# facebookresearch/actionmesh

Hardware: NVIDIA H100
Metric: denoiser_steps_per_sec (higher is better)
Workload: dtype bf16

## Files before the change

actionmesh_b200/csrc/attention.cu:

```cuda
#include "common.cuh"
#include "ptx.cuh"
#include "attention.cuh"

namespace amb {

constexpr int ATT_BQ = 128;
constexpr int ATT_BK = 128;
constexpr int ATT_THREADS = 384;
constexpr int ATT_STAGES = 2;

template <int D>
struct AttnSmem {
  static constexpr int BOX_BYTES = 128 * 128;
  static constexpr int Q_BYTES = (D / 64) * BOX_BYTES;
  static constexpr int KV_BYTES = (D / 64) * BOX_BYTES;
  static constexpr int Q_OFF = 0;
  static constexpr int K_OFF = Q_BYTES;
  static constexpr int V_OFF = K_OFF + ATT_STAGES * KV_BYTES;
  static constexpr int BAR_OFF = V_OFF + ATT_STAGES * KV_BYTES;
  static constexpr int NUM_BARS = 1 + 4 * ATT_STAGES;
  static constexpr int TOTAL = BAR_OFF + NUM_BARS * 8 + 1024;
};

template <int D>
__device__ __forceinline__ void qk_issue(float* sc, uint32_t sq_addr, uint32_t sk_addr) {
#pragma unroll
  for (int k = 0; k < D / 16; ++k) {
    const uint32_t off = (k >> 2) * AttnSmem<D>::BOX_BYTES + (k & 3) * 32;
    wgmma_ss_n128(sc, make_desc_kmajor_sw128(sq_addr + off), make_desc_kmajor_sw128(sk_addr + off), k > 0 ? 1u : 0u);
  }
  wgmma_commit();
}

template <int D>
__device__ __forceinline__ void pv_issue(float* o, const uint32_t* pk, uint32_t sv_addr) {
#pragma unroll
  for (int kk = 0; kk < ATT_BK / 16; ++kk) {
    const uint64_t vdesc = make_desc_mnmajor_sw128(sv_addr + kk * 2048, AttnSmem<D>::BOX_BYTES);
    if constexpr (D == 128) wgmma_rs_n128_tb(o, pk + 4 * kk, vdesc, 1u);
    else wgmma_rs_n64_tb(o, pk + 4 * kk, vdesc, 1u);
  }
  wgmma_commit();
}

__device__ __forceinline__ void softmax_tile(float* sc, int valid, int q, float c, float& m_a, float& m_b, float& l_a,
                                             float& l_b, float& al_a, float& al_b) {
  if (valid < ATT_BK) {
#pragma unroll
    for (int i = 0; i < 16; ++i) {
      const int key = 8 * i + 2 * q;
      if (key >= valid) sc[4 * i] = sc[4 * i + 2] = -INFINITY;
      if (key + 1 >= valid) sc[4 * i + 1] = sc[4 * i + 3] = -INFINITY;
    }
  }
  float mx_a = m_a, mx_b = m_b;
#pragma unroll
  for (int i = 0; i < 16; ++i) {
    mx_a = fmaxf(mx_a, fmaxf(sc[4 * i], sc[4 * i + 1]));
    mx_b = fmaxf(mx_b, fmaxf(sc[4 * i + 2], sc[4 * i + 3]));
  }
  mx_a = fmaxf(mx_a, __shfl_xor_sync(0xffffffffu, mx_a, 1));
  mx_b = fmaxf(mx_b, __shfl_xor_sync(0xffffffffu, mx_b, 1));
  mx_a = fmaxf(mx_a, __shfl_xor_sync(0xffffffffu, mx_a, 2));
  mx_b = fmaxf(mx_b, __shfl_xor_sync(0xffffffffu, mx_b, 2));
  al_a = ex2_approx((m_a - mx_a) * c);
  al_b = ex2_approx((m_b - mx_b) * c);
  m_a = mx_a;
  m_b = mx_b;
  const float mb_a = m_a * c, mb_b = m_b * c;
  float ts_a = 0.f, ts_b = 0.f;
#pragma unroll
  for (int i = 0; i < 16; ++i) {
    sc[4 * i] = ex2_approx(fmaf(sc[4 * i], c, -mb_a));
    sc[4 * i + 1] = ex2_approx(fmaf(sc[4 * i + 1], c, -mb_a));
    sc[4 * i + 2] = ex2_approx(fmaf(sc[4 * i + 2], c, -mb_b));
    sc[4 * i + 3] = ex2_approx(fmaf(sc[4 * i + 3], c, -mb_b));
    ts_a += sc[4 * i] + sc[4 * i + 1];
    ts_b += sc[4 * i + 2] + sc[4 * i + 3];
  }
  l_a = l_a * al_a + ts_a;
  l_b = l_b * al_b + ts_b;
}

__device__ __forceinline__ void pack_p(uint32_t* pk, const float* sc) {
#pragma unroll
  for (int i = 0; i < 16; ++i) {
    pk[2 * i] = pack_bf16(sc[4 * i], sc[4 * i + 1]);
    pk[2 * i + 1] = pack_bf16(sc[4 * i + 2], sc[4 * i + 3]);
  }
}

template <int D>
__global__ void __launch_bounds__(ATT_THREADS, 1)
flash_attn_fwd_kernel(const __grid_constant__ CUtensorMap tmQ, const __grid_constant__ CUtensorMap tmK,
                      const __grid_constant__ CUtensorMap tmV, const AttnParams p) {
  using L = AttnSmem<D>;
  constexpr int DH = D / 64;
  extern __shared__ uint8_t smem_raw[];
  uint8_t* smem = reinterpret_cast<uint8_t*>((reinterpret_cast<uintptr_t>(smem_raw) + 1023) & ~uintptr_t(1023));
  uint64_t* q_full = reinterpret_cast<uint64_t*>(smem + L::BAR_OFF);
  uint64_t* k_full = q_full + 1;
  uint64_t* v_full = k_full + ATT_STAGES;
  uint64_t* k_empty = v_full + ATT_STAGES;
  uint64_t* v_empty = k_empty + ATT_STAGES;

  const int wg = __shfl_sync(0xffffffffu, threadIdx.x >> 7, 0);
  const int warp = threadIdx.x >> 5;
  const int lane = threadIdx.x & 31;
  const int q0 = blockIdx.x * ATT_BQ;
  const int head = blockIdx.y;
  const int batch = blockIdx.z;
  const int tiles_per_chunk = (p.sk_chunk + ATT_BK - 1) / ATT_BK;
  const int n_kv = p.kv_chunks * tiles_per_chunk;

  if (threadIdx.x == 0) {
    tma_prefetch_desc(&tmQ);
    tma_prefetch_desc(&tmK);
    tma_prefetch_desc(&tmV);
    mbar_init(q_full, 1);
    for (int s = 0; s < ATT_STAGES; ++s) {
      mbar_init(&k_full[s], 1);
      mbar_init(&v_full[s], 1);
      mbar_init(&k_empty[s], 8);
      mbar_init(&v_empty[s], 8);
    }
    fence_mbar_init();
  }
  __syncthreads();

  if (wg == 0) {
    reg_dealloc<24>();
    if (warp == 0) {
      if (elect_one()) {
        mbar_expect_tx(q_full, L::Q_BYTES);
        for (int c = 0; c < DH; ++c)
          tma_load_4d(smem + L::Q_OFF + c * L::BOX_BYTES, &tmQ, q_full, c * 64, q0, head, batch, kEvictFirst);
      }
      __syncwarp();
      int s = 0;
      uint32_t phase = 0;
      for (int j = 0; j < n_kv; ++j) {
        const int chunk = j / tiles_per_chunk;
        const int key0 = (j - chunk * tiles_per_chunk) * ATT_BK;
        mbar_wait(&k_empty[s], phase ^ 1);
        if (elect_one()) {
          uint8_t* sk = smem + L::K_OFF + s * L::KV_BYTES;
          mbar_expect_tx(&k_full[s], L::KV_BYTES);
          for (int c = 0; c < DH; ++c)
            tma_load_5d(sk + c * L::BOX_BYTES, &tmK, &k_full[s], c * 64, key0, head, batch, chunk, kEvictLast);
        }
        __syncwarp();
        mbar_wait(&v_empty[s], phase ^ 1);
        if (elect_one()) {
          uint8_t* sv = smem + L::V_OFF + s * L::KV_BYTES;
          mbar_expect_tx(&v_full[s], L::KV_BYTES);
          for (int c = 0; c < DH; ++c)
            tma_load_5d(sv + c * L::BOX_BYTES, &tmV, &v_full[s], c * 64, key0, head, batch, chunk, kEvictLast);
        }
        __syncwarp();
        if (++s == ATT_STAGES) { s = 0; phase ^= 1; }
      }
      for (int j = 0; j < ATT_STAGES; ++j) {
        mbar_wait(&k_empty[s], phase ^ 1);
        mbar_wait(&v_empty[s], phase ^ 1);
        if (++s == ATT_STAGES) { s = 0; phase ^= 1; }
      }
    }
  } else {
    reg_alloc<240>();
    const int q = lane & 3;
    const int r_local = (wg - 1) * 64 + (warp & 3) * 16 + (lane >> 2);
    const uint32_t sq_addr = smem_u32(smem + L::Q_OFF) + (wg - 1) * 64 * 128;
    const uint32_t sk_addr = smem_u32(smem + L::K_OFF);
    const uint32_t sv_addr = smem_u32(smem + L::V_OFF);
    const float c = p.scale_log2;
    const int last_valid = p.sk_chunk - (tiles_per_chunk - 1) * ATT_BK;
    const uint32_t my_turn = wg, other_turn = 3 - wg;

    float o[D / 2];
#pragma unroll
    for (int i = 0; i < D / 2; ++i) o[i] = 0.f;
    float m_a = -INFINITY, m_b = -INFINITY;
    float l_a = 0.f, l_b = 0.f;
    float al_a, al_b;
    float sc[64];
    uint32_t pk[32];

    mbar_wait_watched(q_full, 0);
    mbar_wait_watched(&k_full[0], 0);
    if (wg == 2) named_bar_sync(my_turn, 256);
    wgmma_fence();
    qk_issue<D>(sc, sq_addr, sk_addr);
    named_bar_arrive(other_turn, 256);
    wgmma_wait<0>();
#pragma unroll
    for (int i = 0; i < 64; ++i) reg_fence(sc[i]);
    __syncwarp();
    if (lane == 0) mbar_arrive(&k_empty[0]);
    int jn = tiles_per_chunk == 1 ? 0 : 1;
    softmax_tile(sc, tiles_per_chunk == 1 ? last_valid : ATT_BK, q, c, m_a, m_b, l_a, l_b, al_a, al_b);
    pack_p(pk, sc);

    int s = 0;
    uint32_t phase = 0;
    for (int j = 0; j + 1 < n_kv; ++j) {
      int sn = s + 1;
      uint32_t phn = phase;
      if (sn == ATT_STAGES) { sn = 0; phn ^= 1; }
      mbar_wait_watched(&k_full[sn], phn);
      mbar_wait_watched(&v_full[s], phase);
      named_bar_sync(my_turn, 256);
      wgmma_fence();
      qk_issue<D>(sc, sq_addr, sk_addr + sn * L::KV_BYTES);
      pv_issue<D>(o, pk, sv_addr + s * L::KV_BYTES);
      named_bar_arrive(other_turn, 256);
      wgmma_wait<1>();
#pragma unroll
      for (int i = 0; i < 64; ++i) reg_fence(sc[i]);
      __syncwarp();
      if (lane == 0) mbar_arrive(&k_empty[sn]);
      softmax_tile(sc, jn == tiles_per_chunk - 1 ? last_valid : ATT_BK, q, c, m_a, m_b, l_a, l_b, al_a, al_b);
      if (++jn == tiles_per_chunk) jn = 0;
      wgmma_wait<0>();
#pragma unroll
      for (int i = 0; i < D / 2; ++i) reg_fence(o[i]);
      __syncwarp();
      if (lane == 0) mbar_arrive(&v_empty[s]);
#pragma unroll
      for (int i = 0; i < D / 8; ++i) {
        o[4 * i] *= al_a;
        o[4 * i + 1] *= al_a;
        o[4 * i + 2] *= al_b;
        o[4 * i + 3] *= al_b;
      }
      pack_p(pk, sc);
      s = sn;
      phase = phn;
    }

    mbar_wait_watched(&v_full[s], phase);
    named_bar_sync(my_turn, 256);
    wgmma_fence();
    pv_issue<D>(o, pk, sv_addr + s * L::KV_BYTES);
    if (wg == 1) named_bar_arrive(other_turn, 256);
    wgmma_wait<0>();
#pragma unroll
    for (int i = 0; i < D / 2; ++i) reg_fence(o[i]);
    __syncwarp();
    if (lane == 0) mbar_arrive(&v_empty[s]);

    l_a += __shfl_xor_sync(0xffffffffu, l_a, 1);
    l_b += __shfl_xor_sync(0xffffffffu, l_b, 1);
    l_a += __shfl_xor_sync(0xffffffffu, l_a, 2);
    l_b += __shfl_xor_sync(0xffffffffu, l_b, 2);
    const float inv_a = 1.0f / l_a, inv_b = 1.0f / l_b;
    const int qr_a = q0 + r_local, qr_b = qr_a + 8;
    __nv_bfloat16* obase = p.o + (long long)batch * p.o_stride_b + (long long)head * p.o_stride_h + 2 * q;
#pragma unroll
    for (int i = 0; i < D / 8; ++i) {
      if (qr_a < p.sq)
        *reinterpret_cast<uint32_t*>(obase + (long long)qr_a * p.o_stride_s + 8 * i) = pack_bf16(o[4 * i] * inv_a, o[4 * i + 1] * inv_a);
      if (qr_b < p.sq)
        *reinterpret_cast<uint32_t*>(obase + (long long)qr_b * p.o_stride_s + 8 * i) = pack_bf16(o[4 * i + 2] * inv_b, o[4 * i + 3] * inv_b);
    }
  }
}

template <int D>
static int launch_attn(const amb_attn_args* a, cudaStream_t stream) {
  using L = AttnSmem<D>;
  CUtensorMap tmQ, tmK, tmV;
  int r = encode_attn_maps(a, D, ATT_BQ, ATT_BK, ATT_BK, &tmQ, &tmK, &tmV);
  if (r) return r;
  const AttnParams p = make_attn_params(a);
  dim3 grid((a->sq + ATT_BQ - 1) / ATT_BQ, a->heads, a->batch);
  auto kern = flash_attn_fwd_kernel<D>;
  r = ensure_smem_optin(kern, L::TOTAL);
  if (r) return r;
  kern<<<grid, ATT_THREADS, L::TOTAL, stream>>>(tmQ, tmK, tmV, p);
  AMB_CHECK_CUDA(cudaGetLastError());
  return AMB_OK;
}

}

using namespace amb;

extern "C" int amb_flash_attn_fwd(const amb_attn_args* a, amb_stream_t stream) {
  AMB_CHECK_ARG(a && a->q && a->k && a->v && a->o, "flash_attn: null pointer");
  AMB_CHECK_ARG(a->batch > 0 && a->heads > 0 && a->sq > 0 && a->sk > 0, "flash_attn: bad shape b=%d h=%d sq=%d sk=%d",
                a->batch, a->heads, a->sq, a->sk);
  AMB_CHECK_ARG(a->head_dim == 128 || a->head_dim == 64, "flash_attn: head_dim %d unsupported (64 or 128)", a->head_dim);
  AMB_CHECK_ARG(a->q_stride_s % 8 == 0 && a->k_stride_s % 8 == 0 && a->v_stride_s % 8 == 0 && a->o_stride_s % 8 == 0 &&
                    a->q_stride_h % 8 == 0 && a->k_stride_h % 8 == 0 && a->v_stride_h % 8 == 0 && a->o_stride_h % 8 == 0 &&
                    a->q_stride_b % 8 == 0 && a->k_stride_b % 8 == 0 && a->v_stride_b % 8 == 0 && a->o_stride_b % 8 == 0,
                "flash_attn: strides must be multiples of 8 elements (16 bytes)");
  AMB_CHECK_ARG(a->kv_chunks <= 1 || (a->sk_chunk > 0 && (int64_t)a->sk_chunk * a->kv_chunks == a->sk),
                "flash_attn: kv_chunks * sk_chunk must equal sk");
  AMB_CHECK_ARG(a->batch <= 65535 && a->heads <= 65535, "flash_attn: grid limits");
  cudaStream_t s = (cudaStream_t)stream;
  if (a->head_dim == 64) return launch_attn<64>(a, s);
  return launch_attn<128>(a, s);
}
```

actionmesh_b200/csrc/ptx.cuh:

```cuda
#pragma once
#include <cstdint>
#include <cuda_runtime.h>
#include <cuda_bf16.h>

namespace amb {

__device__ __forceinline__ uint32_t smem_u32(const void* p) {
  return static_cast<uint32_t>(__cvta_generic_to_shared(p));
}
__device__ __forceinline__ uint32_t lane_id() { return threadIdx.x & 31; }

__device__ __forceinline__ bool elect_one() {
  uint32_t pred = 0;
  asm volatile(
      "{\n\t.reg .pred P;\n\t"
      "elect.sync _|P, 0xffffffff;\n\t"
      "selp.u32 %0, 1, 0, P;\n\t}\n"
      : "=r"(pred));
  return pred != 0;
}

__device__ __forceinline__ void mbar_init(uint64_t* bar, uint32_t count) {
  asm volatile("mbarrier.init.shared::cta.b64 [%0], %1;" ::"r"(smem_u32(bar)), "r"(count) : "memory");
}
__device__ __forceinline__ void fence_mbar_init() {
  asm volatile("fence.mbarrier_init.release.cluster;" ::: "memory");
}
__device__ __forceinline__ void fence_proxy_async_smem() {
  asm volatile("fence.proxy.async.shared::cta;" ::: "memory");
}
__device__ __forceinline__ void mbar_expect_tx(uint64_t* bar, uint32_t bytes) {
  asm volatile("mbarrier.arrive.expect_tx.shared::cta.b64 _, [%0], %1;" ::"r"(smem_u32(bar)), "r"(bytes)
               : "memory");
}
__device__ __forceinline__ void mbar_arrive(uint64_t* bar) {
  asm volatile("mbarrier.arrive.shared::cta.b64 _, [%0];" ::"r"(smem_u32(bar)) : "memory");
}
__device__ __forceinline__ uint32_t mbar_try_wait(uint64_t* bar, uint32_t parity) {
  uint32_t ok;
  asm volatile(
      "{\n\t.reg .pred P;\n\t"
      "mbarrier.try_wait.parity.shared::cta.b64 P, [%1], %2;\n\t"
      "selp.u32 %0, 1, 0, P;\n\t}\n"
      : "=r"(ok)
      : "r"(smem_u32(bar)), "r"(parity)
      : "memory");
  return ok;
}
__device__ __forceinline__ void mbar_arrive_cluster(uint64_t* bar, uint32_t cta) {
  asm volatile(
      "{\n\t.reg .b32 ra;\n\t"
      "mapa.shared::cluster.u32 ra, %0, %1;\n\t"
      "mbarrier.arrive.shared::cluster.b64 _, [ra];\n\t}\n"
      ::"r"(smem_u32(bar)), "r"(cta)
      : "memory");
}

__device__ __forceinline__ uint32_t cluster_ctarank() {
  uint32_t r;
  asm volatile("mov.u32 %0, %%cluster_ctarank;" : "=r"(r));
  return r;
}
__device__ __forceinline__ void cluster_sync() {
  asm volatile("barrier.cluster.arrive.release;\n\tbarrier.cluster.wait.acquire;" ::: "memory");
}
__device__ __forceinline__ uint64_t globaltimer_ns() {
  uint64_t t;
  asm volatile("mov.u64 %0, %%globaltimer;" : "=l"(t));
  return t;
}
#ifndef AMB_WAIT_TIMEOUT_NS
#define AMB_WAIT_TIMEOUT_NS 4000000000ull
#endif
#ifndef AMB_WAIT_TIMEOUT_PRINT
#define AMB_WAIT_TIMEOUT_PRINT 0
#endif
__device__ __forceinline__ void mbar_wait(uint64_t* bar, uint32_t parity) {
  if (mbar_try_wait(bar, parity)) return;
  uint64_t t0 = globaltimer_ns();
  uint32_t spins = 0;
  while (!mbar_try_wait(bar, parity)) {
    if ((++spins & 0xfff) == 0 && globaltimer_ns() - t0 > AMB_WAIT_TIMEOUT_NS) {
#if AMB_WAIT_TIMEOUT_PRINT
      printf("amb: mbarrier wait timeout block=(%d,%d,%d) thread=%d bar=%u parity=%u\n", blockIdx.x, blockIdx.y,
             blockIdx.z, threadIdx.x, smem_u32(bar), parity);
#endif
      __trap();
    }
  }
}
__device__ __forceinline__ void mbar_wait_watched(uint64_t* bar, uint32_t parity) {
  while (!mbar_try_wait(bar, parity)) {
  }
}

__device__ __forceinline__ void tma_prefetch_desc(const void* tmap) {
  asm volatile("prefetch.tensormap [%0];" ::"l"(reinterpret_cast<uint64_t>(tmap)) : "memory");
}
constexpr uint64_t kEvictNormal = 0x1000000000000000ull;
constexpr uint64_t kEvictFirst = 0x12F0000000000000ull;
constexpr uint64_t kEvictLast = 0x14F0000000000000ull;

__device__ __forceinline__ void tma_load_2d(void* dst, const void* tmap, uint64_t* bar, int c0, int c1,
                                            uint64_t hint) {
  asm volatile(
      "cp.async.bulk.tensor.2d.shared::cluster.global.mbarrier::complete_tx::bytes.L2::cache_hint"
      " [%0], [%1, {%3, %4}], [%2], %5;"
      :
      : "r"(smem_u32(dst)), "l"(reinterpret_cast<uint64_t>(tmap)), "r"(smem_u32(bar)), "r"(c0), "r"(c1), "l"(hint)
      : "memory");
}
__device__ __forceinline__ void tma_load_2d_multicast(void* dst, const void* tmap, uint64_t* bar, int c0, int c1,
                                                      uint16_t cta_mask, uint64_t hint) {
  asm volatile(
      "cp.async.bulk.tensor.2d.shared::cluster.global.mbarrier::complete_tx::bytes.multicast::cluster.L2::cache_hint"
      " [%0], [%1, {%4, %5}], [%2], %3, %6;"
      :
      : "r"(smem_u32(dst)), "l"(reinterpret_cast<uint64_t>(tmap)), "r"(smem_u32(bar)), "h"(cta_mask), "r"(c0), "r"(c1),
        "l"(hint)
      : "memory");
}
__device__ __forceinline__ void tma_load_4d(void* dst, const void* tmap, uint64_t* bar, int c0, int c1, int c2,
                                            int c3, uint64_t hint) {
  asm volatile(
      "cp.async.bulk.tensor.4d.shared::cluster.global.mbarrier::complete_tx::bytes.L2::cache_hint"
      " [%0], [%1, {%3, %4, %5, %6}], [%2], %7;"
      :
      : "r"(smem_u32(dst)), "l"(reinterpret_cast<uint64_t>(tmap)), "r"(smem_u32(bar)), "r"(c0), "r"(c1), "r"(c2),
        "r"(c3), "l"(hint)
      : "memory");
}

__device__ __forceinline__ void tma_load_5d(void* dst, const void* tmap, uint64_t* bar, int c0, int c1, int c2,
                                            int c3, int c4, uint64_t hint) {
  asm volatile(
      "cp.async.bulk.tensor.5d.shared::cluster.global.mbarrier::complete_tx::bytes.L2::cache_hint"
      " [%0], [%1, {%3, %4, %5, %6, %7}], [%2], %8;"
      :
      : "r"(smem_u32(dst)), "l"(reinterpret_cast<uint64_t>(tmap)), "r"(smem_u32(bar)), "r"(c0), "r"(c1), "r"(c2),
        "r"(c3), "r"(c4), "l"(hint)
      : "memory");
}

__device__ __forceinline__ void wgmma_fence() { asm volatile("wgmma.fence.sync.aligned;" ::: "memory"); }
__device__ __forceinline__ void wgmma_commit() { asm volatile("wgmma.commit_group.sync.aligned;" ::: "memory"); }
template <int N>
__device__ __forceinline__ void wgmma_wait() {
  asm volatile("wgmma.wait_group.sync.aligned %0;" ::"n"(N) : "memory");
}
__device__ __forceinline__ void reg_fence(float& r) { asm volatile("" : "+f"(r)::"memory"); }

__device__ __forceinline__ uint64_t make_smem_desc(uint32_t saddr, uint32_t lbo_bytes, uint32_t sbo_bytes) {
  uint64_t d = 0;
  d |= static_cast<uint64_t>((saddr & 0x3FFFF) >> 4);
  d |= static_cast<uint64_t>((lbo_bytes >> 4) & 0x3FFF) << 16;
  d |= static_cast<uint64_t>((sbo_bytes >> 4) & 0x3FFF) << 32;
  d |= 1ull << 62;
  return d;
}
__device__ __forceinline__ uint64_t make_desc_kmajor_sw128(uint32_t saddr) { return make_smem_desc(saddr, 16, 1024); }
__device__ __forceinline__ uint64_t make_desc_mnmajor_sw128(uint32_t saddr, uint32_t lbo_bytes) {
  return make_smem_desc(saddr, lbo_bytes, 1024);
}

__device__ __forceinline__ void wgmma_ss_n64(float* d, uint64_t desc_a, uint64_t desc_b, uint32_t scale_d) {
  asm volatile(
      "{\n\t.reg .pred p;\n\tsetp.ne.b32 p, %34, 0;\n\t"
      "wgmma.mma_async.sync.aligned.m64n64k16.f32.bf16.bf16 {%0, %1, %2, %3, %4, %5, %6, %7, %8, %9, %10, %11, %12, %13, %14, %15, %16, %17, %18, %19, %20, %21, %22, %23, %24, %25, %26, %27, %28, %29, %30, %31}, %32, %33, p, 1, 1, 0, 0;\n\t}\n"
      : "+f"(d[0]), "+f"(d[1]), "+f"(d[2]), "+f"(d[3]), "+f"(d[4]), "+f"(d[5]), "+f"(d[6]), "+f"(d[7]), "+f"(d[8]), "+f"(d[9]), "+f"(d[10]), "+f"(d[11]), "+f"(d[12]), "+f"(d[13]), "+f"(d[14]), "+f"(d[15]), "+f"(d[16]), "+f"(d[17]), "+f"(d[18]), "+f"(d[19]), "+f"(d[20]), "+f"(d[21]), "+f"(d[22]), "+f"(d[23]), "+f"(d[24]), "+f"(d[25]), "+f"(d[26]), "+f"(d[27]), "+f"(d[28]), "+f"(d[29]), "+f"(d[30]), "+f"(d[31])
      : "l"(desc_a), "l"(desc_b), "r"(scale_d));
}
__device__ __forceinline__ void wgmma_ss_n128(float* d, uint64_t desc_a, uint64_t desc_b, uint32_t scale_d) {
  asm volatile(
      "{\n\t.reg .pred p;\n\tsetp.ne.b32 p, %66, 0;\n\t"
      "wgmma.mma_async.sync.aligned.m64n128k16.f32.bf16.bf16 {%0, %1, %2, %3, %4, %5, %6, %7, %8, %9, %10, %11, %12, %13, %14, %15, %16, %17, %18, %19, %20, %21, %22, %23, %24, %25, %26, %27, %28, %29, %30, %31, %32, %33, %34, %35, %36, %37, %38, %39, %40, %41, %42, %43, %44, %45, %46, %47, %48, %49, %50, %51, %52, %53, %54, %55, %56, %57, %58, %59, %60, %61, %62, %63}, %64, %65, p, 1, 1, 0, 0;\n\t}\n"
      : "+f"(d[0]), "+f"(d[1]), "+f"(d[2]), "+f"(d[3]), "+f"(d[4]), "+f"(d[5]), "+f"(d[6]), "+f"(d[7]), "+f"(d[8]), "+f"(d[9]), "+f"(d[10]), "+f"(d[11]), "+f"(d[12]), "+f"(d[13]), "+f"(d[14]), "+f"(d[15]), "+f"(d[16]), "+f"(d[17]), "+f"(d[18]), "+f"(d[19]), "+f"(d[20]), "+f"(d[21]), "+f"(d[22]), "+f"(d[23]), "+f"(d[24]), "+f"(d[25]), "+f"(d[26]), "+f"(d[27]), "+f"(d[28]), "+f"(d[29]), "+f"(d[30]), "+f"(d[31]), "+f"(d[32]), "+f"(d[33]), "+f"(d[34]), "+f"(d[35]), "+f"(d[36]), "+f"(d[37]), "+f"(d[38]), "+f"(d[39]), "+f"(d[40]), "+f"(d[41]), "+f"(d[42]), "+f"(d[43]), "+f"(d[44]), "+f"(d[45]), "+f"(d[46]), "+f"(d[47]), "+f"(d[48]), "+f"(d[49]), "+f"(d[50]), "+f"(d[51]), "+f"(d[52]), "+f"(d[53]), "+f"(d[54]), "+f"(d[55]), "+f"(d[56]), "+f"(d[57]), "+f"(d[58]), "+f"(d[59]), "+f"(d[60]), "+f"(d[61]), "+f"(d[62]), "+f"(d[63])
      : "l"(desc_a), "l"(desc_b), "r"(scale_d));
}
__device__ __forceinline__ void wgmma_ss_n256(float* d, uint64_t desc_a, uint64_t desc_b, uint32_t scale_d) {
  asm volatile(
      "{\n\t.reg .pred p;\n\tsetp.ne.b32 p, %130, 0;\n\t"
      "wgmma.mma_async.sync.aligned.m64n256k16.f32.bf16.bf16 {%0, %1, %2, %3, %4, %5, %6, %7, %8, %9, %10, %11, %12, %13, %14, %15, %16, %17, %18, %19, %20, %21, %22, %23, %24, %25, %26, %27, %28, %29, %30, %31, %32, %33, %34, %35, %36, %37, %38, %39, %40, %41, %42, %43, %44, %45, %46, %47, %48, %49, %50, %51, %52, %53, %54, %55, %56, %57, %58, %59, %60, %61, %62, %63, %64, %65, %66, %67, %68, %69, %70, %71, %72, %73, %74, %75, %76, %77, %78, %79, %80, %81, %82, %83, %84, %85, %86, %87, %88, %89, %90, %91, %92, %93, %94, %95, %96, %97, %98, %99, %100, %101, %102, %103, %104, %105, %106, %107, %108, %109, %110, %111, %112, %113, %114, %115, %116, %117, %118, %119, %120, %121, %122, %123, %124, %125, %126, %127}, %128, %129, p, 1, 1, 0, 0;\n\t}\n"
      : "+f"(d[0]), "+f"(d[1]), "+f"(d[2]), "+f"(d[3]), "+f"(d[4]), "+f"(d[5]), "+f"(d[6]), "+f"(d[7]), "+f"(d[8]), "+f"(d[9]), "+f"(d[10]), "+f"(d[11]), "+f"(d[12]), "+f"(d[13]), "+f"(d[14]), "+f"(d[15]), "+f"(d[16]), "+f"(d[17]), "+f"(d[18]), "+f"(d[19]), "+f"(d[20]), "+f"(d[21]), "+f"(d[22]), "+f"(d[23]), "+f"(d[24]), "+f"(d[25]), "+f"(d[26]), "+f"(d[27]), "+f"(d[28]), "+f"(d[29]), "+f"(d[30]), "+f"(d[31]), "+f"(d[32]), "+f"(d[33]), "+f"(d[34]), "+f"(d[35]), "+f"(d[36]), "+f"(d[37]), "+f"(d[38]), "+f"(d[39]), "+f"(d[40]), "+f"(d[41]), "+f"(d[42]), "+f"(d[43]), "+f"(d[44]), "+f"(d[45]), "+f"(d[46]), "+f"(d[47]), "+f"(d[48]), "+f"(d[49]), "+f"(d[50]), "+f"(d[51]), "+f"(d[52]), "+f"(d[53]), "+f"(d[54]), "+f"(d[55]), "+f"(d[56]), "+f"(d[57]), "+f"(d[58]), "+f"(d[59]), "+f"(d[60]), "+f"(d[61]), "+f"(d[62]), "+f"(d[63]), "+f"(d[64]), "+f"(d[65]), "+f"(d[66]), "+f"(d[67]), "+f"(d[68]), "+f"(d[69]), "+f"(d[70]), "+f"(d[71]), "+f"(d[72]), "+f"(d[73]), "+f"(d[74]), "+f"(d[75]), "+f"(d[76]), "+f"(d[77]), "+f"(d[78]), "+f"(d[79]), "+f"(d[80]), "+f"(d[81]), "+f"(d[82]), "+f"(d[83]), "+f"(d[84]), "+f"(d[85]), "+f"(d[86]), "+f"(d[87]), "+f"(d[88]), "+f"(d[89]), "+f"(d[90]), "+f"(d[91]), "+f"(d[92]), "+f"(d[93]), "+f"(d[94]), "+f"(d[95]), "+f"(d[96]), "+f"(d[97]), "+f"(d[98]), "+f"(d[99]), "+f"(d[100]), "+f"(d[101]), "+f"(d[102]), "+f"(d[103]), "+f"(d[104]), "+f"(d[105]), "+f"(d[106]), "+f"(d[107]), "+f"(d[108]), "+f"(d[109]), "+f"(d[110]), "+f"(d[111]), "+f"(d[112]), "+f"(d[113]), "+f"(d[114]), "+f"(d[115]), "+f"(d[116]), "+f"(d[117]), "+f"(d[118]), "+f"(d[119]), "+f"(d[120]), "+f"(d[121]), "+f"(d[122]), "+f"(d[123]), "+f"(d[124]), "+f"(d[125]), "+f"(d[126]), "+f"(d[127])
      : "l"(desc_a), "l"(desc_b), "r"(scale_d));
}
__device__ __forceinline__ void wgmma_rs_n64_tb(float* d, const uint32_t* a, uint64_t desc_b, uint32_t scale_d) {
  asm volatile(
      "{\n\t.reg .pred p;\n\tsetp.ne.b32 p, %37, 0;\n\t"
      "wgmma.mma_async.sync.aligned.m64n64k16.f32.bf16.bf16 {%0, %1, %2, %3, %4, %5, %6, %7, %8, %9, %10, %11, %12, %13, %14, %15, %16, %17, %18, %19, %20, %21, %22, %23, %24, %25, %26, %27, %28, %29, %30, %31}, {%32, %33, %34, %35}, %36, p, 1, 1, 1;\n\t}\n"
      : "+f"(d[0]), "+f"(d[1]), "+f"(d[2]), "+f"(d[3]), "+f"(d[4]), "+f"(d[5]), "+f"(d[6]), "+f"(d[7]), "+f"(d[8]), "+f"(d[9]), "+f"(d[10]), "+f"(d[11]), "+f"(d[12]), "+f"(d[13]), "+f"(d[14]), "+f"(d[15]), "+f"(d[16]), "+f"(d[17]), "+f"(d[18]), "+f"(d[19]), "+f"(d[20]), "+f"(d[21]), "+f"(d[22]), "+f"(d[23]), "+f"(d[24]), "+f"(d[25]), "+f"(d[26]), "+f"(d[27]), "+f"(d[28]), "+f"(d[29]), "+f"(d[30]), "+f"(d[31])
      : "r"(a[0]), "r"(a[1]), "r"(a[2]), "r"(a[3]), "l"(desc_b), "r"(scale_d));
}
__device__ __forceinline__ void wgmma_rs_n128_tb(float* d, const uint32_t* a, uint64_t desc_b, uint32_t scale_d) {
  asm volatile(
      "{\n\t.reg .pred p;\n\tsetp.ne.b32 p, %69, 0;\n\t"
      "wgmma.mma_async.sync.aligned.m64n128k16.f32.bf16.bf16 {%0, %1, %2, %3, %4, %5, %6, %7, %8, %9, %10, %11, %12, %13, %14, %15, %16, %17, %18, %19, %20, %21, %22, %23, %24, %25, %26, %27, %28, %29, %30, %31, %32, %33, %34, %35, %36, %37, %38, %39, %40, %41, %42, %43, %44, %45, %46, %47, %48, %49, %50, %51, %52, %53, %54, %55, %56, %57, %58, %59, %60, %61, %62, %63}, {%64, %65, %66, %67}, %68, p, 1, 1, 1;\n\t}\n"
      : "+f"(d[0]), "+f"(d[1]), "+f"(d[2]), "+f"(d[3]), "+f"(d[4]), "+f"(d[5]), "+f"(d[6]), "+f"(d[7]), "+f"(d[8]), "+f"(d[9]), "+f"(d[10]), "+f"(d[11]), "+f"(d[12]), "+f"(d[13]), "+f"(d[14]), "+f"(d[15]), "+f"(d[16]), "+f"(d[17]), "+f"(d[18]), "+f"(d[19]), "+f"(d[20]), "+f"(d[21]), "+f"(d[22]), "+f"(d[23]), "+f"(d[24]), "+f"(d[25]), "+f"(d[26]), "+f"(d[27]), "+f"(d[28]), "+f"(d[29]), "+f"(d[30]), "+f"(d[31]), "+f"(d[32]), "+f"(d[33]), "+f"(d[34]), "+f"(d[35]), "+f"(d[36]), "+f"(d[37]), "+f"(d[38]), "+f"(d[39]), "+f"(d[40]), "+f"(d[41]), "+f"(d[42]), "+f"(d[43]), "+f"(d[44]), "+f"(d[45]), "+f"(d[46]), "+f"(d[47]), "+f"(d[48]), "+f"(d[49]), "+f"(d[50]), "+f"(d[51]), "+f"(d[52]), "+f"(d[53]), "+f"(d[54]), "+f"(d[55]), "+f"(d[56]), "+f"(d[57]), "+f"(d[58]), "+f"(d[59]), "+f"(d[60]), "+f"(d[61]), "+f"(d[62]), "+f"(d[63])
      : "r"(a[0]), "r"(a[1]), "r"(a[2]), "r"(a[3]), "l"(desc_b), "r"(scale_d));
}

__device__ __forceinline__ void named_bar_sync(uint32_t id, uint32_t nthreads) {
  asm volatile("bar.sync %0, %1;" ::"r"(id), "r"(nthreads) : "memory");
}
__device__ __forceinline__ void named_bar_arrive(uint32_t id, uint32_t nthreads) {
  asm volatile("bar.arrive %0, %1;" ::"r"(id), "r"(nthreads) : "memory");
}

template <int N>
__device__ __forceinline__ void reg_alloc() {
  asm volatile("setmaxnreg.inc.sync.aligned.u32 %0;" ::"n"(N));
}
template <int N>
__device__ __forceinline__ void reg_dealloc() {
  asm volatile("setmaxnreg.dec.sync.aligned.u32 %0;" ::"n"(N));
}
__device__ __forceinline__ float ex2_approx(float x) {
  float y;
  asm("ex2.approx.ftz.f32 %0, %1;" : "=f"(y) : "f"(x));
  return y;
}
__device__ __forceinline__ uint32_t pack_bf16(float lo, float hi) {
  __nv_bfloat162 v = __floats2bfloat162_rn(lo, hi);
  return *reinterpret_cast<uint32_t*>(&v);
}
__device__ __forceinline__ float2 unpack_bf16(uint32_t u) {
  __nv_bfloat162 v = *reinterpret_cast<__nv_bfloat162*>(&u);
  return __bfloat1622float2(v);
}

}
```

Measured before the change: 0.7539.

## Share K/V tiles across 2-CTA clusters via TMA multicast in flash attention

Launches the attention kernel as 2-CTA clusters over adjacent query tiles. Each CTA loads half of every K/V tile and multicasts it to both CTAs, which halves per-CTA global/L2 traffic for K and V. The empty barriers now count arrivals from consumers in both CTAs, so the producer must wait for the slower CTA before refilling a stage, and a cluster sync is added at exit. The grid is rounded up to a multiple of the cluster size, which can launch an extra CTA.

```diff
diff --git a/actionmesh_b200/csrc/attention.cu b/actionmesh_b200/csrc/attention.cu
--- a/actionmesh_b200/csrc/attention.cu
+++ b/actionmesh_b200/csrc/attention.cu
@@ -8,12 +8,14 @@
 constexpr int ATT_BK = 128;
 constexpr int ATT_THREADS = 384;
 constexpr int ATT_STAGES = 2;
+constexpr int ATT_CLUSTER = 2;
 
 template <int D>
 struct AttnSmem {
   static constexpr int BOX_BYTES = 128 * 128;
   static constexpr int Q_BYTES = (D / 64) * BOX_BYTES;
   static constexpr int KV_BYTES = (D / 64) * BOX_BYTES;
+  static constexpr int KV_PART_BYTES = BOX_BYTES / ATT_CLUSTER;
   static constexpr int Q_OFF = 0;
   static constexpr int K_OFF = Q_BYTES;
   static constexpr int V_OFF = K_OFF + ATT_STAGES * KV_BYTES;
@@ -91,7 +93,7 @@
 }
 
 template <int D>
-__global__ void __launch_bounds__(ATT_THREADS, 1)
+__global__ void __cluster_dims__(ATT_CLUSTER, 1, 1) __launch_bounds__(ATT_THREADS, 1)
 flash_attn_fwd_kernel(const __grid_constant__ CUtensorMap tmQ, const __grid_constant__ CUtensorMap tmK,
                       const __grid_constant__ CUtensorMap tmV, const AttnParams p) {
   using L = AttnSmem<D>;
@@ -107,6 +109,7 @@
   const int wg = __shfl_sync(0xffffffffu, threadIdx.x >> 7, 0);
   const int warp = threadIdx.x >> 5;
   const int lane = threadIdx.x & 31;
+  const uint32_t rank = cluster_ctarank();
   const int q0 = blockIdx.x * ATT_BQ;
   const int head = blockIdx.y;
   const int batch = blockIdx.z;
@@ -121,12 +124,12 @@
     for (int s = 0; s < ATT_STAGES; ++s) {
       mbar_init(&k_full[s], 1);
       mbar_init(&v_full[s], 1);
-      mbar_init(&k_empty[s], 8);
-      mbar_init(&v_empty[s], 8);
+      mbar_init(&k_empty[s], 8 * ATT_CLUSTER);
+      mbar_init(&v_empty[s], 8 * ATT_CLUSTER);
     }
     fence_mbar_init();
   }
-  __syncthreads();
+  cluster_sync();
 
   if (wg == 0) {
     reg_dealloc<24>();
@@ -139,23 +142,27 @@
       __syncwarp();
       int s = 0;
       uint32_t phase = 0;
+      const uint16_t all_ctas = (uint16_t)((1u << ATT_CLUSTER) - 1);
+      const int part = (int)rank * L::KV_PART_BYTES;
       for (int j = 0; j < n_kv; ++j) {
         const int chunk = j / tiles_per_chunk;
-        const int key0 = (j - chunk * tiles_per_chunk) * ATT_BK;
+        const int key0 = (j - chunk * tiles_per_chunk) * ATT_BK + (int)rank * (ATT_BK / ATT_CLUSTER);
         mbar_wait(&k_empty[s], phase ^ 1);
         if (elect_one()) {
-          uint8_t* sk = smem + L::K_OFF + s * L::KV_BYTES;
+          uint8_t* sk = smem + L::K_OFF + s * L::KV_BYTES + part;
           mbar_expect_tx(&k_full[s], L::KV_BYTES);
           for (int c = 0; c < DH; ++c)
-            tma_load_5d(sk + c * L::BOX_BYTES, &tmK, &k_full[s], c * 64, key0, head, batch, chunk, kEvictLast);
+            tma_load_5d_multicast(sk + c * L::BOX_BYTES, &tmK, &k_full[s], c * 64, key0, head, batch, chunk, all_ctas,
+                                  kEvictLast);
         }
         __syncwarp();
         mbar_wait(&v_empty[s], phase ^ 1);
         if (elect_one()) {
-          uint8_t* sv = smem + L::V_OFF + s * L::KV_BYTES;
+          uint8_t* sv = smem + L::V_OFF + s * L::KV_BYTES + part;
           mbar_expect_tx(&v_full[s], L::KV_BYTES);
           for (int c = 0; c < DH; ++c)
-            tma_load_5d(sv + c * L::BOX_BYTES, &tmV, &v_full[s], c * 64, key0, head, batch, chunk, kEvictLast);
+            tma_load_5d_multicast(sv + c * L::BOX_BYTES, &tmV, &v_full[s], c * 64, key0, head, batch, chunk, all_ctas,
+                                  kEvictLast);
         }
         __syncwarp();
         if (++s == ATT_STAGES) { s = 0; phase ^= 1; }
@@ -196,7 +203,7 @@
 #pragma unroll
     for (int i = 0; i < 64; ++i) reg_fence(sc[i]);
     __syncwarp();
-    if (lane == 0) mbar_arrive(&k_empty[0]);
+    if (lane < ATT_CLUSTER) mbar_arrive_cluster(&k_empty[0], lane);
     int jn = tiles_per_chunk == 1 ? 0 : 1;
     softmax_tile(sc, tiles_per_chunk == 1 ? last_valid : ATT_BK, q, c, m_a, m_b, l_a, l_b, al_a, al_b);
     pack_p(pk, sc);
@@ -218,14 +225,14 @@
 #pragma unroll
       for (int i = 0; i < 64; ++i) reg_fence(sc[i]);
       __syncwarp();
-      if (lane == 0) mbar_arrive(&k_empty[sn]);
+      if (lane < ATT_CLUSTER) mbar_arrive_cluster(&k_empty[sn], lane);
       softmax_tile(sc, jn == tiles_per_chunk - 1 ? last_valid : ATT_BK, q, c, m_a, m_b, l_a, l_b, al_a, al_b);
       if (++jn == tiles_per_chunk) jn = 0;
       wgmma_wait<0>();
 #pragma unroll
       for (int i = 0; i < D / 2; ++i) reg_fence(o[i]);
       __syncwarp();
-      if (lane == 0) mbar_arrive(&v_empty[s]);
+      if (lane < ATT_CLUSTER) mbar_arrive_cluster(&v_empty[s], lane);
 #pragma unroll
       for (int i = 0; i < D / 8; ++i) {
         o[4 * i] *= al_a;
@@ -247,7 +254,7 @@
 #pragma unroll
     for (int i = 0; i < D / 2; ++i) reg_fence(o[i]);
     __syncwarp();
-    if (lane == 0) mbar_arrive(&v_empty[s]);
+    if (lane < ATT_CLUSTER) mbar_arrive_cluster(&v_empty[s], lane);
 
     l_a += __shfl_xor_sync(0xffffffffu, l_a, 1);
     l_b += __shfl_xor_sync(0xffffffffu, l_b, 1);
@@ -264,16 +271,19 @@
         *reinterpret_cast<uint32_t*>(obase + (long long)qr_b * p.o_stride_s + 8 * i) = pack_bf16(o[4 * i + 2] * inv_b, o[4 * i + 3] * inv_b);
     }
   }
+  __syncwarp();
+  cluster_sync();
 }
 
 template <int D>
 static int launch_attn(const amb_attn_args* a, cudaStream_t stream) {
   using L = AttnSmem<D>;
   CUtensorMap tmQ, tmK, tmV;
-  int r = encode_attn_maps(a, D, ATT_BQ, ATT_BK, ATT_BK, &tmQ, &tmK, &tmV);
+  int r = encode_attn_maps(a, D, ATT_BQ, ATT_BK / ATT_CLUSTER, ATT_BK / ATT_CLUSTER, &tmQ, &tmK, &tmV);
   if (r) return r;
   const AttnParams p = make_attn_params(a);
-  dim3 grid((a->sq + ATT_BQ - 1) / ATT_BQ, a->heads, a->batch);
+  const int q_tiles = (a->sq + ATT_BQ - 1) / ATT_BQ;
+  dim3 grid((q_tiles + ATT_CLUSTER - 1) / ATT_CLUSTER * ATT_CLUSTER, a->heads, a->batch);
   auto kern = flash_attn_fwd_kernel<D>;
   r = ensure_smem_optin(kern, L::TOTAL);
   if (r) return r;
diff --git a/actionmesh_b200/csrc/ptx.cuh b/actionmesh_b200/csrc/ptx.cuh
--- a/actionmesh_b200/csrc/ptx.cuh
+++ b/actionmesh_b200/csrc/ptx.cuh
@@ -131,14 +131,14 @@
       : "memory");
 }
 
-__device__ __forceinline__ void tma_load_5d(void* dst, const void* tmap, uint64_t* bar, int c0, int c1, int c2,
-                                            int c3, int c4, uint64_t hint) {
-  asm volatile(
-      "cp.async.bulk.tensor.5d.shared::cluster.global.mbarrier::complete_tx::bytes.L2::cache_hint"
-      " [%0], [%1, {%3, %4, %5, %6, %7}], [%2], %8;"
-      :
-      : "r"(smem_u32(dst)), "l"(reinterpret_cast<uint64_t>(tmap)), "r"(smem_u32(bar)), "r"(c0), "r"(c1), "r"(c2),
-        "r"(c3), "r"(c4), "l"(hint)
+__device__ __forceinline__ void tma_load_5d_multicast(void* dst, const void* tmap, uint64_t* bar, int c0, int c1, int c2,
+                                                      int c3, int c4, uint16_t cta_mask, uint64_t hint) {
+  asm volatile(
+      "cp.async.bulk.tensor.5d.shared::cluster.global.mbarrier::complete_tx::bytes.multicast::cluster.L2::cache_hint"
+      " [%0], [%1, {%4, %5, %6, %7, %8}], [%2], %3, %9;"
+      :
+      : "r"(smem_u32(dst)), "l"(reinterpret_cast<uint64_t>(tmap)), "r"(smem_u32(bar)), "h"(cta_mask), "r"(c0), "r"(c1),
+        "r"(c2), "r"(c3), "r"(c4), "l"(hint)
       : "memory");
 }
 
```

Measured after the change: 0.7755, median of 6. 2.9% higher.
